# jpe17/TwoTowerMLRetrieval

Hardware: AMD Instinct MI355X
Metric: queries/sec top-k over 10M x 256-d docs (higher is better)
Workload: dtype f32 results (bit-identical to the fp32 FMA chain); f16-MFMA screen + fp32 rescoring

## Files before the change

twotowermlretrieval_amd/csrc/score_topk.hip:

```cpp
#include "tt_common.h"

#include <limits.h>
#include <math.h>

namespace {

constexpr int TILE_DOCS = 32;
constexpr int SLAB_BYTES = 32 * 128;
constexpr int NSTAGE = 4;
#ifndef TT_K4_NT_NSTAGE
#define TT_K4_NT_NSTAGE 4
#endif
constexpr int NSTAGE_NT = TT_K4_NT_NSTAGE;
constexpr int WPB = 4;
constexpr int DMA_PER_SLAB = 4;
constexpr int PACE_R = 16;
constexpr int PACE_POLLS = 400;
constexpr int DRAW_POLLS = 1 << 16;
constexpr int DRAW_GAVE_UP = 0x7fffffff;

typedef __attribute__((address_space(3))) void lds_void;
typedef const __attribute__((address_space(1))) void gbl_void;

struct Cand;
// ... 601 lines not shown
        const int64_t ci = pool_i[m];
        if (!ranks_before(pv, pi, cv, ci))
            continue;
        if (bi == INT64_MAX || ranks_before(cv, ci, bv, bi)) {
            bv = cv;
            bi = ci;
        }
    }
#pragma unroll
    for (int off = 32; off >= 1; off >>= 1) {
        const float ov = __shfl_xor(bv, off);
        const int64_t oi = __shfl_xor(bi, off);
        if (oi != INT64_MAX && (bi == INT64_MAX || ranks_before(ov, oi, bv, bi))) {
            bv = ov;
            bi = oi;
        }
    }
    if (lane == 0) {
        red_v[wave] = bv;
        red_i[wave] = bi;
    }
    __syncthreads();
    bv = red_v[0];
    bi = red_i[0];
#pragma unroll
    for (int w = 1; w < MERGE_THREADS / 64; ++w) {
        const float ov = red_v[w];
        const int64_t oi = red_i[w];
        if (oi != INT64_MAX && (bi == INT64_MAX || ranks_before(ov, oi, bv, bi))) {
            bv = ov;
            bi = oi;
        }
    }
    __syncthreads();
}

__global__ __launch_bounds__(MERGE_THREADS) void topk_merge_kernel(const float *__restrict__ in_val,
                                                                   const int64_t *__restrict__ in_idx,
                                                                   int M, int k, float *out_val,
                                                                   int64_t *out_idx, const int *run_if,
                                                                   int seg_len, size_t seg_stride)
{
    if (run_if && run_if[blockIdx.x >> 5] == 0)
        return;
    __shared__ float pool_v[MERGE_POOL];
    __shared__ int64_t pool_i[MERGE_POOL];
    __shared__ float top_v[MERGE_KMAX];
    __shared__ int64_t top_i[MERGE_KMAX];
    __shared__ float red_v[MERGE_THREADS / 64];
    __shared__ int64_t red_i[MERGE_THREADS / 64];
    __shared__ int pool_n;
    const int b = blockIdx.x, tid = threadIdx.x;
    auto v_at = [&](int m) -> float {
        const int sg = m / seg_len, wi = m - sg * seg_len;
        return ((const float *)((const char *)in_val + (size_t)sg * seg_stride))[(size_t)b * seg_len + wi];
    };
    auto ix_at = [&](int m) -> int64_t {
        const int sg = m / seg_len, wi = m - sg * seg_len;
        return ((const int64_t *)((const char *)in_idx + (size_t)sg * seg_stride))[(size_t)b * seg_len + wi];
    };
    if (tid == 0)
        pool_n = 0;
    __syncthreads();

    auto reduce_pool = [&]() {
        const int n = pool_n;
        float pv = INFINITY;
        int64_t pi = -1;
        int kept = 0;
        for (int r = 0; r < k; ++r) {
            float bv;
            int64_t bi;
            pool_next_best(pool_v, pool_i, n, pv, pi, red_v, red_i, bv, bi);
            if (bi == INT64_MAX)
                break;
            if (tid == 0) {
                top_v[r] = bv;
                top_i[r] = bi;
            }
            pv = bv;
            pi = bi;
            kept = r + 1;
        }
        __syncthreads();
        if (tid < kept) {
            pool_v[tid] = top_v[tid];
            pool_i[tid] = top_i[tid];
        }
        if (tid == 0)
            pool_n = kept;
        __syncthreads();
        return kept;
    };

    for (int base = 0; base < M; base += MERGE_SEG) {
        if (pool_n + MERGE_SEG > MERGE_POOL)
            reduce_pool();
        const int end = min(base + MERGE_SEG, M);
        int64_t ci[MERGE_SEG / MERGE_THREADS];
#pragma unroll
        for (int u = 0; u < MERGE_SEG / MERGE_THREADS; ++u) {
            const int m = base + tid + u * MERGE_THREADS;
            ci[u] = m < end ? ix_at(m) : -1;
        }
#pragma unroll
        for (int u = 0; u < MERGE_SEG / MERGE_THREADS; ++u) {
            if (ci[u] >= 0) {
                const int slot = atomicAdd(&pool_n, 1);
                pool_v[slot] = v_at(base + tid + u * MERGE_THREADS);
                pool_i[slot] = ci[u];
            }
        }
        __syncthreads();
    }
    const int kept = reduce_pool();
    if (tid < k) {
        out_val[(size_t)b * k + tid] = tid < kept ? pool_v[tid] : -INFINITY;
        out_idx[(size_t)b * k + tid] = tid < kept ? pool_i[tid] : -1;
    }
}

__device__ __forceinline__ unsigned order_key(float f)
{
    const unsigned b = __float_as_uint(f);
    return (b & 0x80000000u) ? ~b : (b | 0x80000000u);
}

__device__ __forceinline__ float order_key_to_float(unsigned key)
{
    return __uint_as_float((key & 0x80000000u) ? (key & 0x7fffffffu) : ~key);
}

__global__ __launch_bounds__(256) void kth_largest_kernel(const float *__restrict__ vals, int M, int k,
                                                          float *__restrict__ out, const int *run_if,
                                                          float *__restrict__ top_out)
{
    if (run_if && run_if[blockIdx.x >> 5] == 0)
        return;
    __shared__ int hist[256];
    __shared__ int sel[2];
    __shared__ int wpos;
    const int row = blockIdx.x, tid = threadIdx.x, lane = tid & 63;
    const float *v = vals + (size_t)row * M;
    if (M < k) {
        if (tid == 0 && out)
            out[row] = -INFINITY;
        if (top_out)
            for (int i = tid; i < k; i += 256)
                top_out[(size_t)row * k + i] = i < M ? v[i] : -INFINITY;
        return;
    }
    unsigned prefix = 0u, mask = 0u;
    int k_rem = k;
    constexpr int KTH_REG = 16;
    const bool in_regs = M <= 256 * KTH_REG;
    unsigned keys[KTH_REG];
    if (in_regs) {
#pragma unroll
        for (int i = 0; i < KTH_REG; ++i) {
            const int m = tid + 256 * i;
            keys[i] = m < M ? order_key(v[m]) : 0u;
        }
    }
#pragma unroll 1
    for (int pass = 0; pass < 4; ++pass) {
        const int shift = 24 - 8 * pass;
        hist[tid] = 0;
        __syncthreads();
        if (in_regs) {
#pragma unroll
            for (int i = 0; i < KTH_REG; ++i)
                if (tid + 256 * i < M && (keys[i] & mask) == prefix)
                    atomicAdd(&hist[(keys[i] >> shift) & 255u], 1);
        } else {
            for (int m = tid; m < M; m += 256) {
                const unsigned key = order_key(v[m]);
                if ((key & mask) == prefix)
                    atomicAdd(&hist[(key >> shift) & 255u], 1);
            }
        }
        __syncthreads();
        if (tid < 64) {
            int c[4], s = 0;
#pragma unroll
            for (int i = 0; i < 4; ++i) {
                c[i] = hist[255 - (lane * 4 + i)];
                s += c[i];
            }
            int incl = s;
#pragma unroll
            for (int off = 1; off < 64; off <<= 1) {
                const int y = __shfl_up(incl, off);
                if (lane >= off)
                    incl += y;
            }
            int above = incl - s;
#pragma unroll
            for (int i = 0; i < 4; ++i) {
                if (above < k_rem && above + c[i] >= k_rem) {
                    sel[0] = 255 - (lane * 4 + i);
                    sel[1] = above;
                }
                above += c[i];
            }
        }
        __syncthreads();
        prefix |= (unsigned)sel[0] << shift;
        mask |= 0xffu << shift;
        k_rem -= sel[1];
        __syncthreads();
    }
    const float kth = order_key_to_float(prefix);
    if (tid == 0 && out)
        out[row] = kth;
    if (top_out) {
        if (tid == 0)
            wpos = 0;
        __syncthreads();
        float *dst = top_out + (size_t)row * k;
        if (in_regs) {
#pragma unroll
            for (int i = 0; i < KTH_REG; ++i)
                if (tid + 256 * i < M && keys[i] > prefix)
                    dst[atomicAdd(&wpos, 1)] = order_key_to_float(keys[i]);
        } else {
            for (int m = tid; m < M; m += 256)
                if (order_key(v[m]) > prefix)
                    dst[atomicAdd(&wpos, 1)] = v[m];
        }
        for (int i = k - k_rem + tid; i < k; i += 256)
            dst[i] = kth;
    }
}

__global__ __launch_bounds__(256) void score_rank_kernel(const float *__restrict__ Q,
                                                         const float *__restrict__ D, int N, int d,
                                                         const int64_t *__restrict__ target,
                                                         int64_t *rank)
{
    __shared__ float qs[512];
    __shared__ float stage[4][64 * 33];
    __shared__ int cnt[4];
    const int b = blockIdx.x, lane = threadIdx.x & 63, wv = threadIdx.x >> 6;
    const int tg = (int)target[b];
    for (int x = threadIdx.x; x < d; x += 256)
        qs[x] = Q[(size_t)b * d + x];
    __syncthreads();
    float st = 0.0f;
    {
        const float *row = D + (size_t)tg * d;
        for (int x = 0; x < d; ++x)
            st = fmaf(qs[x], row[x], st);
    }
    float *img = stage[wv];
    int c = 0;
    for (int n0 = wv * 64; n0 < N; n0 += 256) {
        float acc = 0.0f;
        for (int x0 = 0; x0 < d; x0 += 32) {
#pragma unroll
            for (int i = 0; i < 8; ++i) {
                const int r = 8 * i + (lane >> 3), n = min(n0 + r, N - 1);
                f32x4 v = {0, 0, 0, 0};
                if (x0 + 4 * (lane & 7) < d)
                    v = *(const f32x4 *)(D + (size_t)n * d + x0 + 4 * (lane & 7));
                float *dst = img + r * 33 + 4 * (lane & 7);
                dst[0] = v.x;
                dst[1] = v.y;
                dst[2] = v.z;
                dst[3] = v.w;
            }
            __builtin_amdgcn_wave_barrier();
            const float *mine = img + lane * 33;
            const int xe = min(32, d - x0);
            for (int x = 0; x < xe; ++x)
                acc = fmaf(qs[x0 + x], mine[x], acc);
            __builtin_amdgcn_wave_barrier();
        }
        const int n = n0 + lane;
        c += (n < N) && (n != tg) && (acc > st || (acc == st && n < tg));
    }
#pragma unroll
    for (int off = 32; off >= 1; off >>= 1)
        c += __shfl_xor(c, off);
    if (lane == 0)
        cnt[wv] = c;
    __syncthreads();
    if (threadIdx.x == 0)
        rank[b] = 1 + (int64_t)cnt[0] + cnt[1] + cnt[2] + cnt[3];
}

__global__ __launch_bounds__(256) void score_all_kernel(const float *__restrict__ Q, const float *__restrict__ D, int N,
                                                        int d, float *__restrict__ S)
{
    __shared__ float qs[512];
    __shared__ float stage[4][64 * 33];
    const int b = blockIdx.y, lane = threadIdx.x & 63, wv = threadIdx.x >> 6;
    for (int x = threadIdx.x; x < d; x += 256)
        qs[x] = Q[(size_t)b * d + x];
    __syncthreads();
    float *img = stage[wv];
    const int n0 = blockIdx.x * 256 + wv * 64;
    if (n0 >= N)
        return;
    float acc = 0.0f;
    for (int x0 = 0; x0 < d; x0 += 32) {
#pragma unroll
        for (int i = 0; i < 8; ++i) {
// ... 508 lines not shown
```

twotowermlretrieval_amd/csrc/screen.hip:

```cpp
#include "tt_common.h"
#include <cmath>

#include <hip/hip_fp16.h>
#include <limits.h>
#include <math.h>

int tt_score_topk_f32_pred(const float *Q, int B, int d, const float *D, int64_t N, int k, int64_t idx_offset,
                           float *out_val, int64_t *out_idx, void *workspace, size_t workspace_bytes,
                           const int *run_if, hipStream_t st);

int tt_kth_largest(const float *vals, int B, int M, int k, float *out, hipStream_t st);
int tt_k_largest_list(const float *vals, int B, int M, int k, float *list, hipStream_t st);

namespace {

typedef _Float16 h8 __attribute__((ext_vector_type(8)));
typedef _Float16 h4 __attribute__((ext_vector_type(4)));
typedef __attribute__((address_space(3))) void lds_void;
typedef const __attribute__((address_space(1))) void gbl_void;

#ifndef TT_SCREEN_STAGGER
#define TT_SCREEN_STAGGER 1
#endif
constexpr int SW = 8;
constexpr int STILE_BYTES = 32 * 512;
constexpr int SRING = 8;
constexpr int STPB = 2;
constexpr int SCAP = 128;
constexpr int SURV_MAX = 1024;
constexpr int POOL_MAX = 8192;
constexpr int FIN_MAX_CHUNKS = 2048;

struct SCand {
    float v;
    int x;
};

__device__ __forceinline__ float screen_eps(float qnorm, float dmax)
{
    return 1.10e-3f * qnorm * dmax + 1e-6f * (qnorm + dmax);
}

__device__ __forceinline__ SCand scand_load_l2(const SCand *p)
{
    unsigned long long u = __hip_atomic_load((const unsigned long long *)p, __ATOMIC_RELAXED, __HIP_MEMORY_SCOPE_AGENT);
    SCand c;
    c.v = __uint_as_float((unsigned)u);
    c.x = (int)(u >> 32);
    return c;
}

struct ScreenParams {
    const float *Q;
    const _Float16 *D16;
    int B, N, k;
    int n_chunks, tiles_per_chunk, n_tiles;
    int static_tiles, tail_g, tail_blocks;
    int *tail_ctr;
    float dmax;
    SCand *cand;
    int *pcnt;
    int *flag;
    float *max_val;
    const float *thr0;
    int thr0_stride;
    const h8 *qimg;
    const float *qnorm;
    const float *dbg_thr;
};

__device__ __forceinline__ void scand_store_async(const SCand *base, unsigned byte_off, float v, int x)
{
    const unsigned long long bits = ((unsigned long long)(unsigned)x << 32) | (unsigned long long)__float_as_uint(v);
    asm volatile("global_store_dwordx2 %0, %1, %2\n\ts_nop 1" ::"v"(byte_off), "v"(bits), "s"(base) : "memory");
}

__device__ __forceinline__ void f32_store_async(float *dst, float v)
{
    asm volatile("global_store_dword %0, %1, off\n\ts_nop 0" ::"v"(dst), "v"(v) : "memory");
}

constexpr int SQUART = SCAP / 4;
constexpr int SQ_TRIGGER = SQUART - 10;
constexpr int SQ_KEEP_MAX = 4 * SQ_TRIGGER - 4;

__device__ __forceinline__ void screen_compact(SCand *base, const int (&n)[4], int k, float slack, int lane, int &n_new,
                                               float &thr_new, bool &have, bool &overflow)
{
    float v[2];
    int x[2], rank[2];
    bool live[2];
#pragma unroll
    for (int i = 0; i < 2; ++i) {
        v[i] = -INFINITY;
        x[i] = INT_MAX;
        rank[i] = 0;
        live[i] = (lane & 31) < ((lane >> 5) ? n[2 * i + 1] : n[2 * i]);
        if (live[i]) {
            const SCand c = scand_load_l2(base + 64 * i + lane);
            v[i] = c.v;
            x[i] = c.x;
        }
    }
#pragma unroll
    for (int i2 = 0; i2 < 2; ++i2) {
#pragma unroll
        for (int sub = 0; sub < 2; ++sub) {
            const int lim = n[2 * i2 + sub];
            for (int l2 = 0; l2 < lim; ++l2) {
                const float sv = __builtin_bit_cast(float, __builtin_amdgcn_readlane(__builtin_bit_cast(int, v[i2]), 32 * sub + l2));
                const int sx = __builtin_amdgcn_readlane(x[i2], 32 * sub + l2);
#pragma unroll
                for (int i = 0; i < 2; ++i)
                    rank[i] += (sv > v[i] || (sv == v[i] && sx < x[i])) ? 1 : 0;
            }
        }
    }
    const int total = n[0] + n[1] + n[2] + n[3];
    have = total >= k;
    overflow = false;
    n_new = total;
    thr_new = -INFINITY;
    if (have) {
        float kth = -INFINITY;
#pragma unroll
        for (int i = 0; i < 2; ++i) {
            const unsigned long long bk = __ballot(live[i] && rank[i] == k - 1);
            if (bk)
                kth = __builtin_bit_cast(float, __builtin_amdgcn_readlane(__builtin_bit_cast(int, v[i]), __ffsll((long long)bk) - 1));
        }
        thr_new = kth - slack;
        n_new = 0;
#pragma unroll
        for (int i = 0; i < 2; ++i)
            n_new += __popcll(__ballot(live[i] && v[i] >= thr_new));
        if (n_new > SQ_KEEP_MAX) {
            overflow = true;
            n_new = k;
        }
    }
#pragma unroll
    for (int i = 0; i < 2; ++i)
        if (live[i] && rank[i] < n_new) {
            SCand c;
            c.v = v[i];
            c.x = x[i];
            base[SQUART * (rank[i] & 3) + (rank[i] >> 2)] = c;
        }
}

__global__ __launch_bounds__(128) void q_image_kernel(const float *__restrict__ Q, int B, h8 *__restrict__ img,
                                                      float *__restrict__ qnorm, int *__restrict__ flag, int n_flags,
                                                      int *__restrict__ tail_ctr, int n_ctr)
{
    __shared__ int any_bad[2];
    if (blockIdx.x == 0)
        for (int i = threadIdx.x; i < n_ctr; i += 128)
            tail_ctr[i] = 0;
    const int lane = threadIdx.x & 63, wv = threadIdx.x >> 6;
    const int S = blockIdx.x * 2 + wv;
    const int g = lane >> 4, n = lane & 15;
    const int qrow = 16 * S + n;
    const bool live = qrow < B;
    const float *qp = Q + (size_t)min(qrow, B - 1) * 256 + 8 * g;
    float ss = 0.0f;
    bool bad = false;
#pragma unroll
    for (int s = 0; s < 8; ++s) {
        const f32x4 a = *(const f32x4 *)(qp + 32 * s);
        const f32x4 b = *(const f32x4 *)(qp + 32 * s + 4);
        h8 hv;
#pragma unroll
        for (int e = 0; e < 4; ++e) {
            const float x0 = live ? a[e] : 0.0f, x1 = live ? b[e] : 0.0f;
            ss += x0 * x0 + x1 * x1;
            bad |= !(fabsf(x0) <= 60000.0f) || !(fabsf(x1) <= 60000.0f);
            hv[e] = (_Float16)x0;
            hv[4 + e] = (_Float16)x1;
        }
        img[((size_t)S * 8 + s) * 64 + lane] = hv;
    }
    ss += __shfl_xor(ss, 16);
    ss += __shfl_xor(ss, 32);
    if (g == 0)
        qnorm[qrow] = sqrtf(ss);
    const bool wave_bad = __ballot(bad && live) != 0ull;
    if (lane == 0)
        any_bad[wv] = wave_bad ? 1 : 0;
    __syncthreads();
    if (threadIdx.x == 0 && (int)blockIdx.x < n_flags)
        flag[blockIdx.x] = (any_bad[0] | any_bad[1]) ? 2 : 0;
}

template <bool MAXONLY, int NSET>
__global__ __launch_bounds__(SW * 64, 2) void screen_kernel(ScreenParams p)
{
    extern __shared__ __attribute__((aligned(16))) char ring[];
    constexpr int DMA_AUX = NSET < 3 ? 2 : 0;
    const int lane = threadIdx.x & 63;
    const int w = __builtin_amdgcn_readfirstlane(threadIdx.x >> 6);
    const int chunk = blockIdx.x % p.n_chunks;
    const int qgroup = blockIdx.x / p.n_chunks;
    int t0 = chunk * p.tiles_per_chunk;
    int t1 = min(t0 + p.tiles_per_chunk, p.static_tiles);
    __shared__ int next_block;
    const int k = p.k;
    const int g = lane >> 4, n = lane & 15;
    constexpr int QW = 16 * NSET, QB = SW * QW;
    const int qbase = qgroup * QB + w * QW;
    const bool wave_live = qbase < p.B;

    h8 qreg[NSET][8];
    float eps2[NSET];
    f32x4 negthr[NSET];
    int cnt[NSET];
#pragma unroll
    for (int c = 0; c < NSET; ++c)
        cnt[c] = 0;
#pragma unroll
    for (int c = 0; c < NSET; ++c) {
        const int qrow = qbase + 16 * c + n;
        const bool live = qrow < p.B;
        float qn = 0.0f;
        if (wave_live) {
            const h8 *src = p.qimg + ((size_t)(qbase / 16 + c) * 8) * 64 + lane;
#pragma unroll
            for (int s = 0; s < 8; ++s)
                qreg[c][s] = src[s * 64];
            qn = p.qnorm[qrow];
        }
        eps2[c] = 2.0f * screen_eps(qn, p.dmax);
        const float floor_thr = -(1.01f * qn * p.dmax + 1e-30f);
        const float t_init = live ? ((!MAXONLY && p.thr0) ? fmaxf(p.thr0[(size_t)qrow * p.thr0_stride + p.thr0_stride - 1] - eps2[c], floor_thr)
                                                    : floor_thr)
                            : INFINITY;
        float c_init = -t_init;
        if (MAXONLY)
            c_init = (p.dbg_thr && live) ? -p.dbg_thr[qrow] : 0.0f;
        negthr[c] = f32x4{c_init, c_init, c_init, c_init};
    }

    SCand *const cwave = p.cand + ((size_t)blockIdx.x * QB + w * QW) * SCAP;

    auto compact_where = [&](int c, unsigned qmask) {
        asm volatile("s_waitcnt vmcnt(0)" ::: "memory");
        while (qmask) {
            const int q = __ffs((int)qmask) - 1;
            qmask &= qmask - 1;
            const int nq[4] = {__builtin_amdgcn_readlane(cnt[c], q), __builtin_amdgcn_readlane(cnt[c], q + 16),
                               __builtin_amdgcn_readlane(cnt[c], q + 32), __builtin_amdgcn_readlane(cnt[c], q + 48)};
            const float slack = __builtin_bit_cast(float, __builtin_amdgcn_readlane(__builtin_bit_cast(int, eps2[c]), q));
            int n_new;
            float tn;
            bool have, ovf;
            screen_compact(cwave + (size_t)(16 * c + q) * SCAP, nq, k, slack, lane, n_new, tn, have, ovf);
            if (ovf && lane == 0)
                atomicOr(p.flag + ((qbase + 16 * c) >> 5), 1);
            if (n == q) {
                cnt[c] = (n_new - g + 3) >> 2;
                if (have)
                    negthr[c] = f32x4{-tn, -tn, -tn, -tn};
            }
        }
    };

    const char *D = (const char *)p.D16;
    const char *rowp[2];
    auto set_rows = [&](int tile) {
#pragma unroll
        for (int i = 0; i < 2; ++i) {
            const int row = 2 * (2 * w + i) + (lane >> 5);
            const int doc = min(tile * 32 + row, p.N - 1);
            const int chunk16 = (lane & 31) ^ (row & 15);
            rowp[i] = D + (size_t)doc * 512 + chunk16 * 16;
        }
    };
    auto dma_issue = [&](int tile, int stage) {
        set_rows(min(tile, t1 - 1));
        char *dst = ring + stage * STILE_BYTES + (2 * w) * 1024;
        __builtin_amdgcn_global_load_lds((gbl_void *)rowp[0], (lds_void *)dst, 16, 0, DMA_AUX);
        __builtin_amdgcn_global_load_lds((gbl_void *)rowp[1], (lds_void *)(dst + 1024), 16, 0, DMA_AUX);
    };
    auto dma_piece = [&](int i, int stage) {
        char *dst = ring + stage * STILE_BYTES + (2 * w + i) * 1024;
        __builtin_amdgcn_global_load_lds((gbl_void *)rowp[i], (lds_void *)dst, 16, 0, DMA_AUX);
    };

    for (;;) {
    if (t0 < t1) {
#pragma unroll
        for (int gi = 0; gi < SRING - STPB; ++gi)
            dma_issue(t0 + gi, gi);
        int stage = 0;
        const int rd_base = n * 512;
        f32x4 acc[2][NSET];
        const bool late = TT_SCREEN_STAGGER && w >= 4;
        bool pending = false;
        int ptile = 0;
        auto epilogue = [&](int tile) {
                const int tile_base = tile * 32;
            const bool partial = tile_base + 32 > p.N;
            if (!MAXONLY) {
                if (partial) {
#pragma unroll
                    for (int u = 0; u < 2; ++u)
#pragma unroll
                        for (int r = 0; r < 4; ++r)
                            if (tile_base + 16 * u + 4 * g + r >= p.N) {
#pragma unroll
                                for (int c = 0; c < NSET; ++c)
                                    acc[u][c][r] = -INFINITY;
                            }
                }
                int mall = INT_MIN;
#pragma unroll
                for (int u = 0; u < 2; ++u)
#pragma unroll
                    for (int c = 0; c < NSET; ++c)
#pragma unroll
                        for (int r = 0; r < 4; ++r)
                            mall = max(mall, __float_as_int(acc[u][c][r]));
                if (__ballot(mall >= 0) != 0ull) {
#pragma unroll
                    for (int c = 0; c < NSET; ++c) {
                        int mu[2];
#pragma unroll
                        for (int u = 0; u < 2; ++u)
                            mu[u] = max(max(__float_as_int(acc[u][c][0]), __float_as_int(acc[u][c][1])),
                                        max(__float_as_int(acc[u][c][2]), __float_as_int(acc[u][c][3])));
                        if (__ballot(max(mu[0], mu[1]) >= 0) == 0ull)
                            continue;
                        const unsigned mine = (unsigned)(((16 * c + n) * SCAP + SQUART * g) * sizeof(SCand));
                        const float thr_c = -negthr[c][0];
#pragma unroll
                        for (int u = 0; u < 2; ++u) {
                            if (__ballot(mu[u] >= 0) == 0ull)
                                continue;
#pragma unroll
                            for (int r = 0; r < 4; ++r) {
                                if (__float_as_int(acc[u][c][r]) >= 0) {
                                    scand_store_async(cwave, mine + (unsigned)cnt[c] * (unsigned)sizeof(SCand),
                                                      acc[u][c][r] + thr_c, tile_base + 16 * u + 4 * g + r);
                                    ++cnt[c];
                                }
                            }
                        }
                        unsigned long long full = __ballot(cnt[c] > SQ_TRIGGER);
                        full = (full | (full >> 32));
                        full = (full | (full >> 16)) & 0xffffull;
                        if (full)
                            compact_where(c, (unsigned)full);
                    }
                }
            } else {
#pragma unroll
                for (int c = 0; c < NSET; ++c) {
                    float m = -INFINITY;
                    if (!partial) {
                        int mi = INT_MIN;
#pragma unroll
                        for (int u = 0; u < 2; ++u)
#pragma unroll
                            for (int r = 0; r < 4; ++r)
                                mi = max(mi, __float_as_int(acc[u][c][r]));
                        m = __int_as_float(mi);
                    } else {
#pragma unroll
                        for (int u = 0; u < 2; ++u)
#pragma unroll
                            for (int r = 0; r < 4; ++r)
                                m = fmaxf(m, tile_base + 16 * u + 4 * g + r < p.N ? acc[u][c][r] : -INFINITY);
                    }
                    m = fmaxf(m, __shfl_xor(m, 16));
                    m = fmaxf(m, __shfl_xor(m, 32));
                    const int qrow = qbase + 16 * c + n;
                    if (g == 0 && qrow < p.B)
                        f32_store_async(p.max_val + (size_t)qrow * p.n_tiles + tile, m);
                }
            }
                };
        for (int tile = t0; tile < t1; ++tile) {
            if ((tile - t0) % STPB == 0) {
                asm volatile("s_waitcnt vmcnt(%0)" ::"n"(2 * (SRING - 2 * STPB)) : "memory");
                __builtin_amdgcn_s_barrier();
            }
            const int fill_stage = (stage + SRING - STPB) % SRING;
            set_rows(min(tile + SRING - STPB, t1 - 1));
            if (!wave_live) {
                dma_piece(0, fill_stage);
                dma_piece(1, fill_stage);
            }
            if (wave_live) {
                if (late && pending)
                    epilogue(ptile);
                const char *buf = ring + stage * STILE_BYTES + rd_base;
                h8 a0[3], a1[3];
                auto a_read = [&](int s) {
                    const int off = ((4 * s + g) ^ n) << 4;
                    a0[s % 3] = *(const h8 *)(buf + off);
                    a1[s % 3] = *(const h8 *)(buf + 16 * 512 + off);
                };
                a_read(0);
                a_read(1);
#pragma unroll
                for (int s = 0; s < 8; ++s) {
                    if (s + 2 < 8)
                        a_read(s + 2);
                    if (s == 2)
                        dma_piece(0, fill_stage);
                    if (s == 6)
                        dma_piece(1, fill_stage);
                    __builtin_amdgcn_sched_barrier(0);
#pragma unroll
                    for (int c = 0; c < NSET; ++c) {
                        const f32x4 c0 = s == 0 ? negthr[c] : acc[0][c];
                        const f32x4 c1 = s == 0 ? negthr[c] : acc[1][c];
                        acc[0][c] = __builtin_amdgcn_mfma_f32_16x16x32_f16(a0[s % 3], qreg[c][s], c0, 0, 0, 0);
                        acc[1][c] = __builtin_amdgcn_mfma_f32_16x16x32_f16(a1[s % 3], qreg[c][s], c1, 0, 0, 0);
                    }
                    __builtin_amdgcn_sched_barrier(0);
                }
                if (late) {
                    pending = true;
                    ptile = tile;
                } else {
                    epilogue(tile);
                }
            }
            stage = (stage + 1) % SRING;
        }
        if (wave_live && late && pending)
            epilogue(ptile);
    }
    if (MAXONLY || p.tail_blocks == 0)
        break;
    asm volatile("s_waitcnt vmcnt(0)" ::: "memory");
    __builtin_amdgcn_s_barrier();
    if (threadIdx.x == 0)
        next_block = atomicAdd(p.tail_ctr + qgroup, 1);
    __syncthreads();
    const int blk = next_block;
    if (blk >= p.tail_blocks)
        break;
    t0 = p.static_tiles + blk * p.tail_g;
    t1 = min(t0 + p.tail_g, p.n_tiles);
    }
    asm volatile("s_waitcnt vmcnt(0)" ::: "memory");
    __builtin_amdgcn_s_barrier();

    if (MAXONLY)
        return;
#pragma unroll
    for (int c = 0; c < NSET; ++c) {
        int tot = cnt[c] + __shfl_xor(cnt[c], 16);
        tot += __shfl_xor(tot, 32);
        const unsigned long long over = __ballot(tot > k) & 0xffffull;
        if (over)
            compact_where(c, (unsigned)over);
        int packed = cnt[c] << (8 * g);
        packed |= __shfl_xor(packed, 16);
        packed |= __shfl_xor(packed, 32);
        const int qrow = qbase + 16 * c + n;
        if (g == 0 && qrow < p.B)
            p.pcnt[(size_t)qrow * p.n_chunks + chunk] = packed;
    }
}

constexpr int TW = 4;
constexpr int TSLAB_BYTES = 32 * 128;
constexpr int TSTAGE = 4;
constexpr int TDMA = 4;
constexpr int TSTREAM_AUX = 2;

template <bool MAXONLY, int NQS = 2>
__global__ __launch_bounds__(TW * 64, 2) void screen_stream_kernel(ScreenParams p)
{
    constexpr int QPT = 16 * NQS;
    extern __shared__ __attribute__((aligned(16))) char ring_all[];
    const int lane = threadIdx.x & 63;
    const int w = __builtin_amdgcn_readfirstlane(threadIdx.x >> 6);
    char *const ring = ring_all + w * (TSTAGE * TSLAB_BYTES);
    const int task = blockIdx.x * TW + w;
    const int n_qtiles = (p.B + QPT - 1) / QPT;
    if (task >= n_qtiles * p.n_chunks)
        return;
    const int qtile = task / p.n_chunks, chunk = task % p.n_chunks;
    const int t0 = chunk * p.tiles_per_chunk;
    const int t1 = min(t0 + p.tiles_per_chunk, p.n_tiles);
    const int k = p.k;
    const int g = lane >> 4, n = lane & 15;
    const int qbase = qtile * QPT;

    h8 qreg[NQS][8];
    float eps2[NQS];
    f32x4 negthr[NQS];
    int cnt[NQS];
#pragma unroll
    for (int c = 0; c < NQS; ++c) {
        cnt[c] = 0;
        const int qrow = qbase + 16 * c + n;
        const bool live = qrow < p.B;
        const h8 *src = p.qimg + ((size_t)(qbase / 16 + c) * 8) * 64 + lane;
#pragma unroll
        for (int s = 0; s < 8; ++s)
            qreg[c][s] = src[s * 64];
        const float qn = p.qnorm[qrow];
        eps2[c] = 2.0f * screen_eps(qn, p.dmax);
        const float floor_thr = -(1.01f * qn * p.dmax + 1e-30f);
        const float t_init = live ? ((!MAXONLY && p.thr0) ? fmaxf(p.thr0[(size_t)qrow * p.thr0_stride + p.thr0_stride - 1] - eps2[c], floor_thr)
                                                    : floor_thr)
                            : INFINITY;
        float c_init = -t_init;
        if (MAXONLY)
            c_init = (p.dbg_thr && live) ? -p.dbg_thr[qrow] : 0.0f;
        negthr[c] = f32x4{c_init, c_init, c_init, c_init};
    }

    SCand *const cwave = p.cand + (size_t)task * QPT * SCAP;

    auto compact_where = [&](int c, unsigned qmask) {
        asm volatile("s_waitcnt vmcnt(0)" ::: "memory");
        while (qmask) {
            const int q = __ffs((int)qmask) - 1;
            qmask &= qmask - 1;
            const int nq[4] = {__builtin_amdgcn_readlane(cnt[c], q), __builtin_amdgcn_readlane(cnt[c], q + 16),
                               __builtin_amdgcn_readlane(cnt[c], q + 32), __builtin_amdgcn_readlane(cnt[c], q + 48)};
            const float slack = __builtin_bit_cast(float, __builtin_amdgcn_readlane(__builtin_bit_cast(int, eps2[c]), q));
            int n_new;
            float tn;
            bool have, ovf;
            screen_compact(cwave + (size_t)(16 * c + q) * SCAP, nq, k, slack, lane, n_new, tn, have, ovf);
            if (ovf && lane == 0)
                atomicOr(p.flag + ((qbase + 16 * c) >> 5), 1);
            if (n == q) {
                cnt[c] = (n_new - g + 3) >> 2;
                if (have)
                    negthr[c] = f32x4{-tn, -tn, -tn, -tn};
            }
        }
    };

    const char *D = (const char *)p.D16;
    int dma_tile = t0, dma_kq = 0;
    const char *rowp[TDMA];
    auto set_rows = [&](int tile) {
#pragma unroll
        for (int jj = 0; jj < TDMA; ++jj) {
            const int row = 8 * jj + (lane >> 3);
            const int doc = min(tile * 32 + row, p.N - 1);
            rowp[jj] = D + (size_t)doc * 512 + (((lane & 7) ^ (row & 7)) << 4);
        }
    };
    auto dma_issue = [&](int stage) {
        char *dst = ring + stage * TSLAB_BYTES;
#pragma unroll
        for (int jj = 0; jj < TDMA; ++jj)
            __builtin_amdgcn_global_load_lds((gbl_void *)(rowp[jj] + dma_kq * 128), (lds_void *)(dst + jj * 1024), 16, 0, TSTREAM_AUX);
        if (++dma_kq == 4) {
            dma_kq = 0;
            dma_tile = min(dma_tile + 1, t1 - 1);
            set_rows(dma_tile);
        }
    };

    if (t0 < t1) {
        set_rows(t0);
#pragma unroll
        for (int i = 0; i < TSTAGE - 1; ++i)
            dma_issue(i);
        int stage = 0;
        const char *rd_row = ring + n * 128;
        const int rsw = n & 7;
        for (int tile = t0; tile < t1; ++tile) {
            f32x4 acc[2][NQS];
#pragma unroll
            for (int kq = 0; kq < 4; ++kq) {
                asm volatile("s_waitcnt vmcnt(%0)" ::"n"(TDMA * (TSTAGE - 2)) : "memory");
                const char *buf = rd_row + stage * TSLAB_BYTES;
                h8 a[2][2];
#pragma unroll
                for (int s2 = 0; s2 < 2; ++s2)
#pragma unroll
                    for (int u = 0; u < 2; ++u)
                        a[u][s2] = *(const h8 *)(buf + u * 2048 + (((4 * s2 + g) ^ rsw) << 4));
                asm volatile("s_waitcnt lgkmcnt(0)" ::: "memory");
                dma_issue((stage + TSTAGE - 1) % TSTAGE);
#pragma unroll
                for (int s2 = 0; s2 < 2; ++s2)
#pragma unroll
                    for (int c = 0; c < NQS; ++c)
#pragma unroll
                        for (int u = 0; u < 2; ++u) {
                            const f32x4 cin = (kq == 0 && s2 == 0) ? negthr[c] : acc[u][c];
                            acc[u][c] = __builtin_amdgcn_mfma_f32_16x16x32_f16(a[u][s2], qreg[c][2 * kq + s2], cin, 0, 0, 0);
                        }
                stage = (stage + 1) % TSTAGE;
            }
            const int tile_base = tile * 32;
            const bool partial = tile_base + 32 > p.N;
            if (!MAXONLY) {
                if (partial) {
// ... 313 lines not shown
            const f32x4 v = *(const f32x4 *)(D + row * d + x);
            h4 hv;
#pragma unroll
            for (int e = 0; e < 4; ++e) {
                ss += v[e] * v[e];
                amax = fmaxf(amax, fabsf(v[e]));
                if (!(fabsf(v[e]) <= 3.0e38f))
                    amax = INFINITY;
                hv[e] = (_Float16)v[e];
            }
            *(h4 *)(out + row * d + x) = hv;
        }
#pragma unroll
        for (int off = 32; off >= 1; off >>= 1)
            ss += __shfl_xor(ss, off);
        nmax = fmaxf(nmax, sqrtf(ss));
    }
#pragma unroll
    for (int off = 32; off >= 1; off >>= 1)
        amax = fmaxf(amax, __shfl_xor(amax, off));
    if (lane == 0) {
        red[wave] = nmax;
        red[4 + wave] = amax;
    }
    __syncthreads();
    if (threadIdx.x == 0) {
        atomicMax(stats, __float_as_uint(fmaxf(fmaxf(red[0], red[1]), fmaxf(red[2], red[3]))));
        atomicMax(stats + 1, __float_as_uint(fmaxf(fmaxf(red[4], red[5]), fmaxf(red[6], red[7]))));
    }
}

__global__ __launch_bounds__(256) void build_from_bf16_kernel(const unsigned short *__restrict__ S, int64_t N, int d,
                                                              float *__restrict__ out32, _Float16 *__restrict__ out16,
                                                              unsigned *__restrict__ stats)
{
    __shared__ float red[8];
    const int lane = threadIdx.x & 63, wave = threadIdx.x >> 6;
    float nmax = 0.0f, amax = 0.0f;
    for (int64_t row = (int64_t)blockIdx.x * 4 + wave; row < N; row += (int64_t)gridDim.x * 4) {
        float ss = 0.0f;
        for (int x = lane * 4; x < d; x += 256) {
            const uint2 raw = *(const uint2 *)(S + row * d + x);
            f32x4 v;
            v[0] = __uint_as_float(raw.x << 16);
            v[1] = __uint_as_float(raw.x & 0xffff0000u);
            v[2] = __uint_as_float(raw.y << 16);
            v[3] = __uint_as_float(raw.y & 0xffff0000u);
            h4 hv;
#pragma unroll
            for (int e = 0; e < 4; ++e) {
                ss += v[e] * v[e];
                amax = fmaxf(amax, fabsf(v[e]));
                if (!(fabsf(v[e]) <= 3.0e38f))
                    amax = INFINITY;
                hv[e] = (_Float16)v[e];
            }
            *(f32x4 *)(out32 + row * d + x) = v;
            if (out16)
                *(h4 *)(out16 + row * d + x) = hv;
        }
#pragma unroll
        for (int off = 32; off >= 1; off >>= 1)
            ss += __shfl_xor(ss, off);
        nmax = fmaxf(nmax, sqrtf(ss));
    }
#pragma unroll
    for (int off = 32; off >= 1; off >>= 1)
        amax = fmaxf(amax, __shfl_xor(amax, off));
    if (lane == 0) {
        red[wave] = nmax;
        red[4 + wave] = amax;
    }
    __syncthreads();
    if (threadIdx.x == 0 && stats) {
        atomicMax(stats, __float_as_uint(fmaxf(fmaxf(red[0], red[1]), fmaxf(red[2], red[3]))));
        atomicMax(stats + 1, __float_as_uint(fmaxf(fmaxf(red[4], red[5]), fmaxf(red[6], red[7]))));
    }
}

struct SPlan {
    bool stream;
    int nset;
    int n_qgroups;
    int q_per_block;
    int n_tiles, n_chunks, tiles_per_chunk;
    int static_tiles, tail_g, tail_blocks;
    size_t tailctr_off;
    bool sample;
    int s_tiles, s_chunks, s_tiles_per_chunk;
    int64_t s_docs;
    size_t cand_off, pcnt_off, smax_val_off, sthr_val_off, qimg_off, qnorm_off, stats_off, ws_bytes;
    int rows_pad;
};

constexpr int64_t SAMPLE_MIN_N = 65536;
constexpr int STREAM_MAX_B = 64;

int one_round(bool stream, int n_qgroups)
{
    return stream ? (tt_device_cus() * 2 * TW + n_qgroups - 1) / n_qgroups : (tt_device_cus() + n_qgroups - 1) / n_qgroups;
}

SPlan make_splan(int B, int64_t N, int k)
{
    SPlan pl;
    pl.stream = B <= STREAM_MAX_B;
    if (B <= SW * 32) {
        pl.nset = B <= SW * 16 ? 1 : 2;
    } else {
        const int groups = (B + SW * 64 - 1) / (SW * 64);
        pl.nset = (B + groups - 1) / groups <= SW * 48 ? 3 : 4;
    }
    pl.q_per_block = pl.stream ? (B <= 32 ? 32 : 64) : SW * 16 * pl.nset;
    pl.n_qgroups = (B + pl.q_per_block - 1) / pl.q_per_block;
    pl.n_tiles = (int)((N + 31) / 32);
    int max_chunks = pl.stream && N >= SAMPLE_MIN_N ? FIN_MAX_CHUNKS : POOL_MAX / (k + 16);
    if (!pl.stream)
        max_chunks = max_chunks > 255 ? 255 : max_chunks;
    const TTChunks c = tt_chunks(pl.n_tiles, one_round(pl.stream, pl.n_qgroups), max_chunks);
    pl.n_chunks = c.n_chunks;
    const TTTailSplit t = tt_tail_split(c.tiles_per_chunk, c.n_chunks, pl.n_tiles,
                                        pl.stream ? 0 : TT_AB_SWITCH(TT_SCREEN_TAIL_DIV, 8), 16, 8, 32);
    pl.tiles_per_chunk = t.own;
    pl.static_tiles = t.static_tiles;
    pl.tail_g = t.tail_g;
    pl.tail_blocks = t.tail_blocks;
    const int n_tasks = pl.n_qgroups * pl.n_chunks;
    const size_t rows = (size_t)pl.n_qgroups * pl.q_per_block;
    pl.rows_pad = (int)rows;
    pl.sample = N >= SAMPLE_MIN_N;
    int64_t s_docs = N / 64;
    const int per_k = k <= 16 ? 4096 : 2048;
    const int64_t s_min = (int64_t)k * per_k < N / 4 ? (int64_t)k * per_k : N / 4;
    s_docs = s_docs < s_min ? s_min : s_docs;
    s_docs = s_docs < 32 ? 32 : s_docs;
    pl.s_docs = (s_docs + 31) / 32 * 32;
    pl.s_tiles = (int)(pl.s_docs / 32);
    const TTChunks sc = tt_chunks(pl.s_tiles, one_round(pl.stream, pl.n_qgroups), INT_MAX);
    pl.s_tiles_per_chunk = sc.tiles_per_chunk;
    pl.s_chunks = pl.sample ? sc.n_chunks : 0;
    TTWorkspace ws;
    pl.cand_off = ws.take((size_t)n_tasks * pl.q_per_block * SCAP * sizeof(SCand));
    pl.pcnt_off = ws.take(rows * pl.n_chunks * sizeof(int));
    pl.smax_val_off = ws.take(rows * (size_t)(pl.sample ? pl.s_tiles : 1) * sizeof(float));
    pl.sthr_val_off = ws.take(rows * sizeof(float));
    pl.qimg_off = ws.take(rows * 256 * sizeof(_Float16));
    pl.qnorm_off = ws.take(rows * sizeof(float));
    pl.tailctr_off = ws.take((size_t)pl.n_qgroups * sizeof(int));
    pl.stats_off = ws.take(rows * 2 * sizeof(int));
    pl.ws_bytes = ws.off;
    return pl;
}

template <bool MAXONLY>
const void *screen_fn(bool stream, int q_per_block, int nset)
{
    if (stream)
        return q_per_block == 64 ? (const void *)screen_stream_kernel<MAXONLY, 4> : (const void *)screen_stream_kernel<MAXONLY, 2>;
    switch (nset) {
    case 4: return (const void *)screen_kernel<MAXONLY, 4>;
    case 3: return (const void *)screen_kernel<MAXONLY, 3>;
    case 2: return (const void *)screen_kernel<MAXONLY, 2>;
    default: return (const void *)screen_kernel<MAXONLY, 1>;
    }
}

int launch_screen(bool stream, int q_per_block, int nset, bool maxonly, ScreenParams p, int n_tasks, hipStream_t st)
{
    const void *fn = maxonly ? screen_fn<true>(stream, q_per_block, nset) : screen_fn<false>(stream, q_per_block, nset);
    const size_t lds = stream ? (size_t)TW * TSTAGE * TSLAB_BYTES : (size_t)SRING * STILE_BYTES;
    const int blocks = stream ? (n_tasks + TW - 1) / TW : n_tasks;
    TT_HIP_CHECK(hipFuncSetAttribute(fn, hipFuncAttributeMaxDynamicSharedMemorySize, (int)lds));
    void *args[] = {&p};
    TT_HIP_CHECK(hipLaunchKernel(fn, dim3(blocks), dim3((stream ? TW : SW) * 64), args, lds, st));
    return TT_OK;
}

}

TT_EXPORT int tt_index_build_f16(const float *D, int64_t N, int d, void *D16, float *stats, tt_stream_t stream)
{
    if (N < 0 || d <= 0 || (d & 3))
        return tt_fail(TT_ERR_BAD_SHAPE, "tt_index_build_f16: N=%lld d=%d", (long long)N, d);
    if (!stats || (N > 0 && (!D || !D16)))
        return tt_fail(TT_ERR_BAD_SHAPE, "tt_index_build_f16: null pointer");
    hipStream_t st = (hipStream_t)stream;
    TT_RC_CHECK(tt_zero_async(stats, 2 * sizeof(float), st));
    if (N == 0)
        return TT_OK;
    const int64_t want_blocks = (N + 3) / 4;
    hipLaunchKernelGGL(build_f16_kernel, dim3((unsigned)(want_blocks > 8192 ? 8192 : want_blocks)), dim3(256), 0, st, D,
                       N, d, (_Float16 *)D16, (unsigned *)stats);
    TT_LAUNCH_CHECK();
    return TT_OK;
}

TT_EXPORT int tt_index_build_from_bf16(const void *D_bf16, int64_t N, int d, float *D32, void *D16, float *stats,
                                       int reset_stats, tt_stream_t stream)
{
    if (N < 0 || d <= 0 || (d & 3))
        return tt_fail(TT_ERR_BAD_SHAPE, "tt_index_build_from_bf16: N=%lld d=%d", (long long)N, d);
    if (N > 0 && (!D_bf16 || !D32))
        return tt_fail(TT_ERR_BAD_SHAPE, "tt_index_build_from_bf16: null pointer");
    hipStream_t st = (hipStream_t)stream;
    if (stats && reset_stats)
        TT_RC_CHECK(tt_zero_async(stats, 2 * sizeof(float), st));
    if (N == 0)
        return TT_OK;
    const int64_t want_blocks = (N + 3) / 4;
    hipLaunchKernelGGL(build_from_bf16_kernel, dim3((unsigned)(want_blocks > 8192 ? 8192 : want_blocks)), dim3(256), 0,
                       st, (const unsigned short *)D_bf16, N, d, D32, (_Float16 *)D16, (unsigned *)stats);
    TT_LAUNCH_CHECK();
    return TT_OK;
}

TT_EXPORT size_t tt_score_topk_screened_workspace_bytes(int B, int64_t N, int d, int k)
{
    if (B <= 0 || N <= 0)
        return 0;
    return make_splan(B, N, k).ws_bytes + tt_score_topk_workspace_bytes(B, N, d, k);
}

TT_EXPORT size_t tt_score_topk_screened_stats_offset(int B, int64_t N, int d, int k)
{
    (void)d;
    if (B <= 0 || N <= 0)
        return 0;
    return make_splan(B, N, k).stats_off;
}

namespace {
__global__ void seed_fill_kernel(float *seed, int n)
{
    const int i = blockIdx.x * 256 + threadIdx.x;
    if (i < n)
        seed[i] = -3.0e38f;
}

enum class Phase {
    Whole,
    SeedThreshold,
    SeedList,
    Seeded,
};

int screened_impl(const char *who, Phase phase, const float *Q, int B, int d, const float *D32, const void *D16, int64_t N, int k,
                  int k_seed, float dmax_norm, int64_t idx_offset, float *out_val, int64_t *out_idx, int32_t *fallback_flag,
                  float *seed, void *workspace, size_t workspace_bytes, void *const *prof_events, hipStream_t st)
{
    if (B <= 0 || N <= 0 || k <= 0)
        return tt_fail(TT_ERR_BAD_SHAPE, "%s: B=%d N=%lld k=%d", who, B, (long long)N, k);
    if (d != 256)
        return tt_fail(TT_ERR_UNSUPPORTED, "%s: d=%d (supported: 256)", who, d);
    if (k > 64)
        return tt_fail(TT_ERR_UNSUPPORTED, "%s: k=%d > 64", who, k);
    if (N >= (int64_t)INT_MAX - 64)
        return tt_fail(TT_ERR_UNSUPPORTED, "%s: N too large; shard the corpus", who);
    if (!(dmax_norm >= 0.0f) || !(dmax_norm < 60000.0f))
        return tt_fail(TT_ERR_UNSUPPORTED, "%s: corpus norm %g outside the fp16 range", who, dmax_norm);
    const bool seed_only = phase == Phase::SeedThreshold || phase == Phase::SeedList;
    const bool caller_seed = phase == Phase::Seeded;
    if (!Q || !D16 || !fallback_flag || (!seed_only && (!D32 || !out_val || !out_idx)) || (phase != Phase::Whole && !seed))
        return tt_fail(TT_ERR_BAD_SHAPE, "%s: null pointer", who);
    if (seed_only && (k_seed < 1 || k_seed > k))
        return tt_fail(TT_ERR_BAD_SHAPE, "%s: k_seed=%d outside [1, k=%d]", who, k_seed, k);
    const SPlan pl = make_splan(B, N, k);
    const size_t need = pl.ws_bytes + tt_score_topk_workspace_bytes(B, N, d, k);
    if (!workspace || workspace_bytes < need || ((uintptr_t)workspace & 255))
        return tt_fail(TT_ERR_WORKSPACE, "%s: workspace %zu < %zu bytes", who, workspace_bytes, need);
    char *ws = (char *)workspace;
    const int k_thr = phase == Phase::SeedThreshold ? k_seed : k;
    float *thr_out = phase == Phase::SeedThreshold ? seed : (float *)(ws + pl.sthr_val_off);

    ScreenParams sp;
    sp.Q = Q;
    sp.D16 = (const _Float16 *)D16;
    sp.B = B;
    sp.N = (int)N;
    sp.k = k;
    sp.n_chunks = pl.n_chunks;
    sp.tiles_per_chunk = pl.tiles_per_chunk;
    sp.n_tiles = pl.n_tiles;
    sp.static_tiles = pl.static_tiles;
    sp.tail_g = pl.tail_g;
    sp.tail_blocks = pl.tail_blocks;
    sp.tail_ctr = (int *)(ws + pl.tailctr_off);
    sp.dmax = dmax_norm;
    sp.cand = (SCand *)(ws + pl.cand_off);
    sp.pcnt = (int *)(ws + pl.pcnt_off);
    sp.flag = fallback_flag;
    sp.max_val = nullptr;
    sp.thr0 = nullptr;
    sp.thr0_stride = k;
    sp.qimg = (const h8 *)(ws + pl.qimg_off);
    sp.qnorm = (const float *)(ws + pl.qnorm_off);
    sp.dbg_thr = nullptr;
    if (caller_seed) {
        sp.thr0 = seed;
        sp.thr0_stride = 1;
    } else {
        hipLaunchKernelGGL(q_image_kernel, dim3(pl.rows_pad / 32), dim3(128), 0, st, Q, B, (h8 *)(ws + pl.qimg_off),
                           (float *)(ws + pl.qnorm_off), fallback_flag, (B + 31) / 32, (int *)(ws + pl.tailctr_off),
                           pl.n_qgroups);
        TT_LAUNCH_CHECK();
        if (pl.sample) {
            ScreenParams ss = sp;
            ss.N = (int)pl.s_docs;
            ss.n_tiles = pl.s_tiles;
            ss.n_chunks = pl.s_chunks;
            ss.tiles_per_chunk = pl.s_tiles_per_chunk;
            ss.static_tiles = pl.s_tiles;
            ss.tail_blocks = 0;
            ss.max_val = (float *)(ws + pl.smax_val_off);
            TT_RC_CHECK(launch_screen(pl.stream, pl.q_per_block, pl.nset, true, ss, pl.n_qgroups * pl.s_chunks, st));
            if (phase == Phase::SeedList)
                TT_RC_CHECK(tt_k_largest_list(ss.max_val, B, pl.s_tiles, k_seed, seed, st));
            else
                TT_RC_CHECK(tt_kth_largest(ss.max_val, B, pl.s_tiles, k_thr, thr_out, st));
            sp.thr0 = (const float *)(ws + pl.sthr_val_off);
            sp.thr0_stride = 1;
        } else if (seed_only) {
            const int n = phase == Phase::SeedList ? B * k_seed : B;
            hipLaunchKernelGGL(seed_fill_kernel, dim3((n + 255) / 256), dim3(256), 0, st, seed, n);
// ... 143 lines not shown
```

Baseline: 263,500.

## Add opt-in flag-based LDS ring sync to screen kernel and retune ring

```diff
diff --git a/twotowermlretrieval_amd/csrc/score_topk.hip b/twotowermlretrieval_amd/csrc/score_topk.hip
--- a/twotowermlretrieval_amd/csrc/score_topk.hip
+++ b/twotowermlretrieval_amd/csrc/score_topk.hip
@@ -777,7 +777,7 @@
     }
     unsigned prefix = 0u, mask = 0u;
     int k_rem = k;
-    constexpr int KTH_REG = 16;
+    constexpr int KTH_REG = 20;
     const bool in_regs = M <= 256 * KTH_REG;
     unsigned keys[KTH_REG];
     if (in_regs) {
diff --git a/twotowermlretrieval_amd/csrc/screen.hip b/twotowermlretrieval_amd/csrc/screen.hip
--- a/twotowermlretrieval_amd/csrc/screen.hip
+++ b/twotowermlretrieval_amd/csrc/screen.hip
@@ -24,8 +24,22 @@
 #endif
 constexpr int SW = 8;
 constexpr int STILE_BYTES = 32 * 512;
-constexpr int SRING = 8;
-constexpr int STPB = 2;
+#ifndef TT_SCREEN_SRING
+#define TT_SCREEN_SRING 8
+#endif
+#ifndef TT_SCREEN_STPB
+#define TT_SCREEN_STPB 1
+#endif
+constexpr int SRING = TT_SCREEN_SRING;
+constexpr int STPB = TT_SCREEN_STPB;
+static_assert(SRING >= 2 * STPB && SRING <= 9, "ring: two intervals in LDS, at most 9 x 16 KiB");
+constexpr int SPF = SRING - STPB;
+#ifndef TT_SCREEN_RING_DEFAULT
+#define TT_SCREEN_RING_DEFAULT 0
+#endif
+constexpr int SRING_F = SPF + 3 < 9 ? SPF + 3 : 9;
+constexpr int SSIG = SPF - 4 > 2 ? SPF - 4 : 2;
+constexpr int SRING_SPIN_MAX = 1 << 20;
 constexpr int SCAP = 128;
 constexpr int SURV_MAX = 1024;
 constexpr int POOL_MAX = 8192;
@@ -43,7 +57,8 @@
 
 __device__ __forceinline__ SCand scand_load_l2(const SCand *p)
 {
-    unsigned long long u = __hip_atomic_load((const unsigned long long *)p, __ATOMIC_RELAXED, __HIP_MEMORY_SCOPE_AGENT);
+    unsigned long long u;
+    asm volatile("global_load_dwordx2 %0, %1, off sc1\n\ts_waitcnt vmcnt(0)" : "=v"(u) : "v"(p) : "memory");
     SCand c;
     c.v = __uint_as_float((unsigned)u);
     c.x = (int)(u >> 32);
@@ -192,10 +207,19 @@
         flag[blockIdx.x] = (any_bad[0] | any_bad[1]) ? 2 : 0;
 }
 
-template <bool MAXONLY, int NSET>
+template <bool MAXONLY, int NSET, bool FLAGS = false>
 __global__ __launch_bounds__(SW * 64, 2) void screen_kernel(ScreenParams p)
 {
+    constexpr int RING = FLAGS ? SRING_F : SRING;
     extern __shared__ __attribute__((aligned(16))) char ring[];
+    __shared__ int ring_full[FLAGS ? SRING_F : 1], ring_free[FLAGS ? SRING_F : 1];
+    if (FLAGS) {
+        if (threadIdx.x < RING) {
+            ring_full[threadIdx.x] = 0;
+            ring_free[threadIdx.x] = 0;
+        }
+        __syncthreads();
+    }
     constexpr int DMA_AUX = NSET < 3 ? 2 : 0;
     const int lane = threadIdx.x & 63;
     const int w = __builtin_amdgcn_readfirstlane(threadIdx.x >> 6);
@@ -286,12 +310,68 @@
         __builtin_amdgcn_global_load_lds((gbl_void *)rowp[i], (lds_void *)dst, 16, 0, DMA_AUX);
     };
 
+    int rslot = 0, ruse = 0, sslot = 0, sig = 0;
+    bool ring_expired = false;
+    auto lds_addr = [](int *ctr) { return (unsigned)(size_t)(__attribute__((address_space(3))) int *)ctr; };
+    auto ring_wait = [&](int *ctr, int target) {
+        const unsigned a = lds_addr(ctr);
+        for (int spins = 0;; ++spins) {
+            int v;
+            asm volatile("ds_read_b32 %0, %1\n\ts_waitcnt lgkmcnt(0)" : "=v"(v) : "v"(a) : "memory");
+            if (__builtin_amdgcn_readfirstlane(v) >= target)
+                break;
+            if (spins == SRING_SPIN_MAX) {
+                ring_expired = true;
+                break;
+            }
+            __builtin_amdgcn_s_sleep(1);
+        }
+    };
+    auto ring_add = [&](int *ctr) {
+        if (lane == 0)
+            asm volatile("ds_add_u32 %0, %1" ::"v"(lds_addr(ctr)), "v"(1) : "memory");
+    };
+    auto wait_free = [&](int slot, int use) { ring_wait(ring_free + slot, SW * use); };
+    auto publish = [&](int tile) {
+        const int upto = min(tile + SSIG, t1 - 1);
+        if (sig > upto)
+            return;
+        switch (min(tile + SPF - 1, t1 - 1) - upto) {
+        case 0: asm volatile("s_waitcnt vmcnt(0)" ::: "memory"); break;
+        case 1: asm volatile("s_waitcnt vmcnt(2)" ::: "memory"); break;
+        case 2: asm volatile("s_waitcnt vmcnt(4)" ::: "memory"); break;
+        default: asm volatile("s_waitcnt vmcnt(6)" ::: "memory"); break;
+        }
+        static_assert(SPF - 1 - SSIG <= 3, "publish: vmcnt cases");
+        for (; sig <= upto; ++sig) {
+            ring_add(ring_full + sslot);
+            sslot = sslot + 1 == RING ? 0 : sslot + 1;
+        }
+    };
+
     for (;;) {
     if (t0 < t1) {
-#pragma unroll
-        for (int gi = 0; gi < SRING - STPB; ++gi)
-            dma_issue(t0 + gi, gi);
         int stage = 0;
+        if (FLAGS) {
+            stage = rslot;
+            sig = t0;
+            int slot = rslot, use = ruse;
+#pragma unroll
+            for (int gi = 0; gi < SPF; ++gi) {
+                if (t0 + gi < t1) {
+                    wait_free(slot, use);
+                    dma_issue(t0 + gi, slot);
+                }
+                if (++slot == RING) {
+                    slot = 0;
+                    ++use;
+                }
+            }
+        } else {
+#pragma unroll
+            for (int gi = 0; gi < SPF; ++gi)
+                dma_issue(t0 + gi, gi);
+        }
         const int rd_base = n * 512;
         f32x4 acc[2][NSET];
         const bool late = TT_SCREEN_STAGGER && w >= 4;
@@ -380,19 +460,35 @@
             }
                 };
         for (int tile = t0; tile < t1; ++tile) {
-            if ((tile - t0) % STPB == 0) {
+            if (!FLAGS && (tile - t0) % STPB == 0) {
                 asm volatile("s_waitcnt vmcnt(%0)" ::"n"(2 * (SRING - 2 * STPB)) : "memory");
                 __builtin_amdgcn_s_barrier();
             }
-            const int fill_stage = (stage + SRING - STPB) % SRING;
-            set_rows(min(tile + SRING - STPB, t1 - 1));
+            if (FLAGS)
+                publish(tile);
+            const int fill_stage = stage + SPF < RING ? stage + SPF : stage + SPF - RING;
+            const int fill_use = stage + SPF < RING ? ruse : ruse + 1;
+            const bool fill = !FLAGS || tile + SPF < t1;
+            if (fill)
+                set_rows(min(tile + SPF, t1 - 1));
             if (!wave_live) {
-                dma_piece(0, fill_stage);
-                dma_piece(1, fill_stage);
+                if (FLAGS && fill)
+                    wait_free(fill_stage, fill_use);
+                if (fill) {
+                    dma_piece(0, fill_stage);
+                    dma_piece(1, fill_stage);
+                }
+                if (FLAGS)
+                    ring_add(ring_free + stage);
             }
             if (wave_live) {
                 if (late && pending)
                     epilogue(ptile);
+                if (FLAGS) {
+                    ring_wait(ring_full + stage, SW * (ruse + 1));
+                    if (fill)
+                        wait_free(fill_stage, fill_use);
+                }
                 const char *buf = ring + stage * STILE_BYTES + rd_base;
                 h8 a0[3], a1[3];
                 auto a_read = [&](int s) {
@@ -406,9 +502,11 @@
                 for (int s = 0; s < 8; ++s) {
                     if (s + 2 < 8)
                         a_read(s + 2);
-                    if (s == 2)
+                    if (FLAGS && s == 5)
+                        ring_add(ring_free + stage);
+                    if (fill && s == 2)
                         dma_piece(0, fill_stage);
-                    if (s == 6)
+                    if (fill && s == 6)
                         dma_piece(1, fill_stage);
                     __builtin_amdgcn_sched_barrier(0);
 #pragma unroll
@@ -427,10 +525,14 @@
                     epilogue(tile);
                 }
             }
-            stage = (stage + 1) % SRING;
+            if (++stage == RING) {
+                stage = 0;
+                ++ruse;
+            }
         }
         if (wave_live && late && pending)
             epilogue(ptile);
+        rslot = stage;
     }
     if (MAXONLY || p.tail_blocks == 0)
         break;
@@ -447,6 +549,11 @@
     }
     asm volatile("s_waitcnt vmcnt(0)" ::: "memory");
     __builtin_amdgcn_s_barrier();
+    if (FLAGS && ring_expired && lane == 0) {
+        const int f1 = min((qgroup + 1) * QB, p.B + 31) >> 5;
+        for (int f = (qgroup * QB) >> 5; f < f1; ++f)
+            atomicOr(p.flag + f, 1);
+    }
 
     if (MAXONLY)
         return;
@@ -1066,23 +1173,25 @@
     return pl;
 }
 
-template <bool MAXONLY>
+template <bool MAXONLY, bool FLAGS>
 const void *screen_fn(bool stream, int q_per_block, int nset)
 {
     if (stream)
         return q_per_block == 64 ? (const void *)screen_stream_kernel<MAXONLY, 4> : (const void *)screen_stream_kernel<MAXONLY, 2>;
     switch (nset) {
-    case 4: return (const void *)screen_kernel<MAXONLY, 4>;
-    case 3: return (const void *)screen_kernel<MAXONLY, 3>;
-    case 2: return (const void *)screen_kernel<MAXONLY, 2>;
-    default: return (const void *)screen_kernel<MAXONLY, 1>;
+    case 4: return (const void *)screen_kernel<MAXONLY, 4, FLAGS>;
+    case 3: return (const void *)screen_kernel<MAXONLY, 3, FLAGS>;
+    case 2: return (const void *)screen_kernel<MAXONLY, 2, FLAGS>;
+    default: return (const void *)screen_kernel<MAXONLY, 1, FLAGS>;
     }
 }
 
 int launch_screen(bool stream, int q_per_block, int nset, bool maxonly, ScreenParams p, int n_tasks, hipStream_t st)
 {
-    const void *fn = maxonly ? screen_fn<true>(stream, q_per_block, nset) : screen_fn<false>(stream, q_per_block, nset);
-    const size_t lds = stream ? (size_t)TW * TSTAGE * TSLAB_BYTES : (size_t)SRING * STILE_BYTES;
+    const bool flags = TT_AB_SWITCH(TT_SCREEN_RING, TT_SCREEN_RING_DEFAULT) != 0;
+    const void *fn = flags ? (maxonly ? screen_fn<true, true>(stream, q_per_block, nset) : screen_fn<false, true>(stream, q_per_block, nset))
+                           : (maxonly ? screen_fn<true, false>(stream, q_per_block, nset) : screen_fn<false, false>(stream, q_per_block, nset));
+    const size_t lds = stream ? (size_t)TW * TSTAGE * TSLAB_BYTES : (size_t)(flags ? SRING_F : SRING) * STILE_BYTES;
     const int blocks = stream ? (n_tasks + TW - 1) / TW : n_tasks;
     TT_HIP_CHECK(hipFuncSetAttribute(fn, hipFuncAttributeMaxDynamicSharedMemorySize, (int)lds));
     void *args[] = {&p};
```

After: 274,200 (median of 6 runs). +4.0%, better.
